# mfkiwl/msckf_stereo_c

Measured on AMD Instinct MI355X. Metric: stereo frames/sec/node on EuRoC-shape input; ATE RMSE vs CPU ref, higher is better.
Workload: dtype f64

## Files before the change

### msckf_stereo_c_amd/csrc/hip/ekf_linalg.hip

```cpp
#include <mutex>
#include <type_traits>
#include "ekf_device.h"
#include "ekf_cap.h"
#include "chol_block.h"

typedef double v4f64 __attribute__((ext_vector_type(4)));

__device__ __forceinline__ bool ekf_direct_wanted(const EkfStreamDev &S) { return ekf_mode_direct(S.qr_mode, S.rows_out[EKF_ROWS_STACKED], S.rows_out[EKF_ROWS_NA]); }
__device__ __forceinline__ bool ekf_skip_gram(const EkfStreamDev &S) { return ekf_mode_householder(S.qr_mode) || ekf_direct_wanted(S); }
__device__ __forceinline__ bool ekf_direct(const EkfStreamDev &S) { return (S.rows_out[EKF_ROWS_DIAG] & EKF_DIAG_DIRECT) != 0; }
__device__ __forceinline__ bool ekf_row_has(unsigned long long rm, int clone) { return clone < 0 ? rm != 0ULL : ((rm >> clone) & 1ULL) != 0ULL; }

template <int MODE> struct GemmTraits;
template <> struct GemmTraits<GM_GRAM> { static constexpr bool TA = true,  SYM = true,  KMIN_I = false, KMIN_J = false; };
template <> struct GemmTraits<GM_T>    { static constexpr bool TA = true,  SYM = false, KMIN_I = true,  KMIN_J = false; };
template <> struct GemmTraits<GM_S2>   { static constexpr bool TA = false, SYM = true,  KMIN_I = false, KMIN_J = true;  };
template <> struct GemmTraits<GM_PUPD> { static constexpr bool TA = true,  SYM = true,  KMIN_I = false, KMIN_J = false; };

#define GT EKF_GEMM_TILE
#ifndef GK
#define GK 32
#endif
#define GNE (GK / 8)

template <int MODE>
__global__ __launch_bounds__(256) void k_ekf_gemm(const EkfStreamDev *streams) {
    using TR = GemmTraits<MODE>;
    const EkfStreamDev &S = streams[blockIdx.y];
    if (S.n_feat <= 0) return;
    if (MODE != GM_PUPD && (S.route & EKF_ROUTE_SMALL)) return;
    const int d = S.d, ld = S.ld;
    int gram_tile_i = 0, gram_tile_j = 0;
    EkfCapResult cap = {0, 0, 0, 0ULL};
    if (MODE == GM_GRAM) {
        int tg = 1;
        while ((tg + 1) * (tg + 1) <= (int)gridDim.x) ++tg;
        gram_tile_i = (int)blockIdx.x / tg; gram_tile_j = (int)blockIdx.x - gram_tile_i * tg;
        if (gram_tile_j > gram_tile_i || gram_tile_i * GT > S.na_max) return;
        cap = ekf_cap_local(S, blockIdx.x == 0);
        if (ekf_mode_householder(S.qr_mode) || ekf_mode_direct(S.qr_mode, cap.stacked, cap.na)) return;
    }
    const int na = MODE == GM_GRAM ? cap.na : S.rows_out[EKF_ROWS_NA];
    const int *__restrict__ act = S.act;
    const double *__restrict__ A; const double *__restrict__ B; double *C;
    int M, N, K;
    double alpha = 1.0, beta = 0.0, diag_add = 0.0;
    if (MODE == GM_GRAM)      { A = S.Hs; B = S.Hs; C = S.S; M = N = na + 1; K = cap.end; }
    const int nk = MODE == GM_GRAM ? 0 : S.rows_out[EKF_ROWS_NK];
    const bool direct = MODE != GM_GRAM && MODE != GM_PUPD && ekf_direct(S);
    if (MODE == GM_T)         { A = direct ? S.Hs : S.S;  B = S.P;  C = S.T; M = nk; N = d; K = na; }
    else if (MODE == GM_S2)   { A = S.T;  B = direct ? S.Hs : S.S;  C = S.W; M = N = nk; K = na; diag_add = S.sigma2; }
    else if (MODE == GM_PUPD) { A = S.T;  B = S.T;  C = S.P; M = N = d; K = nk; alpha = -1.0; beta = 1.0; }
    const int tiles_n = (N + GT - 1) / GT, tiles_m = (M + GT - 1) / GT;
    const int tile = blockIdx.x;
    if (MODE == GM_PUPD && tile >= tiles_m * tiles_n) {
        const int c0 = (tile - tiles_m * tiles_n) * GT;
        if (c0 >= d) return;
        const double *Y = S.T;
        __shared__ double s_part[8][GT + 1];
        const int cl = threadIdx.x & 31, ks = threadIdx.x >> 5;
        const int c = c0 + cl;
        double s2 = 0;
        if (c < d)
            for (int k = ks; k < nk; k += 8) s2 += Y[(size_t)k * ld + c] * Y[(size_t)k * ld + d];
        s_part[ks][cl] = s2;
        __syncthreads();
        if (ks == 0 && c < d) {
            double t = 0;
#pragma unroll
            for (int q = 0; q < 8; ++q) t += s_part[q][cl];
            S.delta_x[c] = t;
        }
        return;
    }
    if (MODE != GM_GRAM && tile >= tiles_m * tiles_n) return;
    const int ti = MODE == GM_GRAM ? gram_tile_i : tile / tiles_n, tj = MODE == GM_GRAM ? gram_tile_j : tile - ti * tiles_n;
    if (MODE == GM_GRAM && ti >= tiles_m) return;
    if (TR::SYM && tj > ti) return;
    const int i0 = ti * GT, j0 = tj * GT;
    __shared__ double sA[GK][GT + 1];
    __shared__ double sB[GK][GT + 1];
    const int tid = threadIdx.x, lane = tid & 63, wave = tid >> 6;
    const int wi = (wave >> 1) * 16, wj = (wave & 1) * 16;
    const int lo = tid & 31, hi = tid >> 5;
    int k_begin = 0;
    if (TR::KMIN_I && !direct) k_begin = (i0 / GK) * GK;
    if (TR::KMIN_J && !direct) k_begin = (j0 / GK) * GK;
    const int k_end = K;
    int colA = i0 + lo, colB = j0 + lo;
    if (MODE == GM_GRAM) {
        colA = (i0 + lo < na) ? ekf_act_column(cap.clones, i0 + lo) : d;
        colB = (j0 + lo < na) ? ekf_act_column(cap.clones, j0 + lo) : d;
    }
    const int cloneA = MODE == GM_GRAM ? (colA < d ? (colA - EKF_IMU_DIM) / 6 : -1) : 0;
    const int cloneB = MODE == GM_GRAM ? (colB < d ? (colB - EKF_IMU_DIM) / 6 : -1) : 0;
    const unsigned long long *__restrict__ rowmask = S.rowmask;
    const int *__restrict__ rowidx = S.act + S.ld;
    double ra[GNE], rb[GNE];
    auto fetch = [&](int k0) {
#pragma unroll
        for (int e = 0; e < GNE; ++e) {
            if (MODE == GM_GRAM) {
                const int gk = k0 + hi + 8 * e;
                double v = 0.0, w = 0.0;
                if (gk < K) {
                    const unsigned long long rm = rowmask[gk];
                    const bool onA = ekf_row_has(rm, cloneA), onB = ekf_row_has(rm, cloneB);
                    if (onA && i0 + lo < M) v = A[(size_t)gk * ld + colA];
                    if (onB && j0 + lo < N) w = B[(size_t)gk * ld + colB];
                }
                ra[e] = v; rb[e] = w;
                continue;
            }
            const int ii = TR::TA ? lo : hi + 8 * (e / (GK / 32)), kk = TR::TA ? hi + 8 * e : lo + 32 * (e % (GK / 32));
            const int gi = i0 + ii, gk = k0 + kk;
            double v = 0.0;
            if (gi < M && gk < K && !(TR::KMIN_I && !direct && gk < gi)) {
                if (MODE == GM_S2) v = A[(size_t)gi * ld + act[gk]];
                else if (MODE == GM_T && direct) {
                    const int col = act[gk], ri = rowidx[gi];
                    if ((rowmask[ri] >> ((col - EKF_IMU_DIM) / 6)) & 1ULL) v = A[(size_t)ri * ld + col];
                }
                else v = A[(size_t)gk * ld + (MODE == GM_GRAM ? colA : gi)];
            }
            ra[e] = v;
            const int gj = j0 + lo, gkb = k0 + hi + 8 * e;
            double w = 0.0;
            if (gj < N && gkb < K && !(TR::KMIN_J && !direct && gkb < gj)) {
                if (MODE == GM_T) w = B[(size_t)act[gkb] * ld + gj];
                else if (MODE == GM_S2 && direct) {
                    const int col = act[gkb], rj = rowidx[gj];
                    if ((rowmask[rj] >> ((col - EKF_IMU_DIM) / 6)) & 1ULL) w = B[(size_t)rj * ld + col];
                }
                else w = B[(size_t)gkb * ld + (MODE == GM_GRAM ? colB : gj)];
            }
            rb[e] = w;
        }
    };
    v4f64 acc = {0.0, 0.0, 0.0, 0.0};
    if (k_begin < k_end) fetch(k_begin);
    for (int k0 = k_begin; k0 < k_end; k0 += GK) {
        __syncthreads();
#pragma unroll
        for (int e = 0; e < GNE; ++e) {
            if (TR::TA) sA[hi + 8 * e][lo] = ra[e]; else sA[lo + 32 * (e % (GK / 32))][hi + 8 * (e / (GK / 32))] = ra[e];
            sB[hi + 8 * e][lo] = rb[e];
        }
        __syncthreads();
        if (k0 + GK < k_end) fetch(k0 + GK);
#pragma unroll
        for (int s = 0; s < GK / 4; ++s) {
            const int kk = 4 * s + (lane >> 4);
            const double a = sA[kk][wi + (lane & 15)];
            const double b = sB[kk][wj + (lane & 15)];
            acc = __builtin_amdgcn_mfma_f64_16x16x4f64(a, b, acc, 0, 0, 0);
        }
    }
#pragma unroll
    for (int r = 0; r < 4; ++r) {
        const int i = i0 + wi + (lane >> 4) + 4 * r;
        const int j = j0 + wj + (lane & 15);
        if (i >= M || j >= N) continue;
        if (TR::SYM && j > i) continue;
        double v = alpha * acc[r];
        if (MODE == GM_PUPD) v += beta * C[(size_t)i * ld + j];
        if (i == j) v += diag_add;
        C[(size_t)i * ld + j] = v;
        if (TR::SYM && i != j) C[(size_t)j * ld + i] = v;
        if (MODE == GM_PUPD && i == j && i >= 12 && i < 15 && S.pos_var_out) S.pos_var_out[i - 12] = v;
    }
}

template <int Q> __device__ __forceinline__ double qr_lane_sum(double v) {
    auto bfly = [](double x, auto ctrl) {
        const long long b = __double_as_longlong(x);
        const int lo = __builtin_amdgcn_update_dpp(0, (int)b, decltype(ctrl)::value, 0xf, 0xf, true);
        const int hi = __builtin_amdgcn_update_dpp(0, (int)(b >> 32), decltype(ctrl)::value, 0xf, 0xf, true);
        return x + __longlong_as_double(((long long)hi << 32) | (unsigned int)lo);
    };
    v = bfly(v, std::integral_constant<int, 0xB1>());
    v = bfly(v, std::integral_constant<int, 0x4E>());
    if (Q == 8) v = bfly(v, std::integral_constant<int, 0x141>());
    return v;
}
template <int Q, int RL, class ColOf, class RAt>
__device__ __forceinline__ void tsqr_wide(const EkfStreamDev &S, int n1, int K, ColOf colOf, RAt Rat, double *sB) {
    constexpr int BR = Q * RL;
    const int tid = threadIdx.x, nth = blockDim.x, ld = S.ld;
    const int q = tid & (Q - 1), g = tid / Q, ng = nth / Q;
    for (int k0 = 0; k0 < K; k0 += BR) {
        __syncthreads();
        for (int e = tid; e < BR * n1; e += nth) {
            const int r = e / n1, c = e - r * n1, gk = k0 + r;
            double v = 0.0;
            if (gk < K) {
                int col, clone;
                colOf(c, col, clone);
                if (ekf_row_has(S.rowmask[gk], clone)) v = S.Hs[(size_t)gk * ld + col];
            }
            sB[e] = v;
        }
        __syncthreads();
        double *own = sB + (size_t)q * RL * n1;
        for (int k = 0; k < n1; ++k) {
            double bk[RL];
            double ss = 0.0;
#pragma unroll
            for (int i = 0; i < RL; ++i) { bk[i] = own[i * n1 + k]; ss += bk[i] * bk[i]; }
            ss = qr_lane_sum<Q>(ss);
            const double x0 = Rat(k, k);
            if (ss < 1e-200 || ss < 1e-40 * (x0 * x0)) continue;
            const double nrm = sqrt(x0 * x0 + ss);
            const double alpha = x0 > 0.0 ? -nrm : nrm;
            const double v0 = x0 - alpha;
            const double beta = 2.0 / (v0 * v0 + ss);
            for (int j = k + 1 + g; j < n1; j += ng) {
                double bj[RL];
                double dot = 0.0;
#pragma unroll
                for (int i = 0; i < RL; ++i) { bj[i] = own[i * n1 + j]; dot += bk[i] * bj[i]; }
                const double rkj = Rat(k, j);
                const double t = beta * (qr_lane_sum<Q>(dot) + v0 * rkj);
#pragma unroll
                for (int i = 0; i < RL; ++i) own[i * n1 + j] = bj[i] - t * bk[i];
                if (q == 0) Rat(k, j) = rkj - t * v0;
            }
            __syncthreads();
            if (tid == 0) Rat(k, k) = alpha;
        }
    }
    __syncthreads();
}
template <class ColOf, class RAt>
__device__ __forceinline__ void tsqr_quads(const EkfStreamDev &S, int n1, int K, ColOf colOf, RAt Rat, double *sB, int room) {
    if (room >= 48 * n1) tsqr_wide<4, 12>(S, n1, K, colOf, Rat, sB);
    else if (room >= 32 * n1) tsqr_wide<4, 8>(S, n1, K, colOf, Rat, sB);
    else tsqr_wide<4, 4>(S, n1, K, colOf, Rat, sB);
}

__device__ __forceinline__ int ekf_compress_entry(const EkfStreamDev &S, int *s_w ) {
    const int na = S.rows_out[EKF_ROWS_NA], me = S.rows_out[EKF_ROWS_END], d = S.d, ld = S.ld;
    if (na <= 0) { if (threadIdx.x == 0) S.rows_out[EKF_ROWS_DIAG] = 0; return 1; }
    if (ekf_direct_wanted(S)) {
        int *rowidx = S.act + ld;
        const int tid = threadIdx.x, lane = tid & 63, wave = tid >> 6, nw = (int)blockDim.x >> 6;
        int base = 0;
        for (int r0 = 0; r0 < me; r0 += (int)blockDim.x) {
            const int r = r0 + tid;
            const bool on = r < me && S.rowmask[r] != 0ULL;
            const unsigned long long b = __ballot(on);
            if (lane == 0) s_w[wave] = __popcll(b);
            __syncthreads();
            int off = base, tot = 0;
            for (int w = 0; w < nw; ++w) { const int c = s_w[w]; if (w < wave) off += c; tot += c; }
            if (on && off + __popcll(b & ((1ULL << lane) - 1ULL)) < ld) rowidx[off + __popcll(b & ((1ULL << lane) - 1ULL))] = r;
            base += tot;
            __syncthreads();
        }
        __threadfence_block();
        __syncthreads();
        for (int i = tid; i < base; i += (int)blockDim.x) S.T[(size_t)i * ld + d] = S.Hs[(size_t)rowidx[i] * ld + d];
        if (tid == 0) { S.rows_out[EKF_ROWS_DIAG] = EKF_DIAG_DIRECT; S.rows_out[EKF_ROWS_NK] = base; }
        return 1;
    }
    return ekf_skip_gram(S) ? 2 : 0;
}
template <class RAt>
__device__ __forceinline__ void ekf_hand_over_r(const EkfStreamDev &S, int na, RAt Rat, int diag) {
    const int tid = threadIdx.x, nth = blockDim.x, d = S.d, ld = S.ld;
    for (int e = tid; e < na * na; e += nth) {
        const int i = e / na, j = e - i * na;
        if (j <= i) S.S[(size_t)i * ld + j] = Rat(j, i);
    }
    for (int k = tid; k < na; k += nth) S.T[(size_t)k * ld + d] = Rat(k, na);
    if (tid == 0) S.rows_out[EKF_ROWS_DIAG] = diag | EKF_DIAG_HOUSEHOLDER;
}
template <class RAt>
__device__ __forceinline__ void ekf_compress_exit(const EkfStreamDev &S, bool gram_done, int diag, RAt Rat, double *sB, int room) {
    const int na = S.rows_out[EKF_ROWS_NA], n1 = na + 1, K = S.rows_out[EKF_ROWS_END], d = S.d;
    const int tid = threadIdx.x, nth = blockDim.x;
    if (!ekf_mode_redo_householder(S.qr_mode, gram_done, (diag & EKF_DIAG_BIAS) != 0)) { if (tid == 0) S.rows_out[EKF_ROWS_DIAG] = diag; return; }
    __syncthreads();
    for (int e = tid; e < n1 * n1; e += nth) { const int k = e / n1, j = e - k * n1; if (j >= k) Rat(k, j) = 0.0; }
    const int *act = S.act;
    tsqr_quads(S, n1, K, [=](int c, int &col, int &clone) { col = c < na ? act[c] : d; clone = c < na ? (col - EKF_IMU_DIM) / 6 : -1; }, Rat, sB, room);
    ekf_hand_over_r(S, na, Rat, diag);
}


__device__ __forceinline__ double tq_rows_sum(double v) {
    {
        const unsigned long long b = (unsigned long long)__double_as_longlong(v);
        const auto lo = __builtin_amdgcn_permlane16_swap((unsigned)b, (unsigned)b, false, false), hi = __builtin_amdgcn_permlane16_swap((unsigned)(b >> 32), (unsigned)(b >> 32), false, false);
        v = __longlong_as_double((long long)(((unsigned long long)hi[0] << 32) | lo[0])) + __longlong_as_double((long long)(((unsigned long long)hi[1] << 32) | lo[1]));
    }
    {
        const unsigned long long b = (unsigned long long)__double_as_longlong(v);
        const auto lo = __builtin_amdgcn_permlane32_swap((unsigned)b, (unsigned)b, false, false), hi = __builtin_amdgcn_permlane32_swap((unsigned)(b >> 32), (unsigned)(b >> 32), false, false);
        v = __longlong_as_double((long long)(((unsigned long long)hi[0] << 32) | lo[0])) + __longlong_as_double((long long)(((unsigned long long)hi[1] << 32) | lo[1]));
    }
    return v;
}
__device__ __forceinline__ double tq_rcp(double x) {
    double r = __builtin_amdgcn_rcp(x);
    r = __builtin_fma(__builtin_fma(-x, r, 1.0), r, r);
    r = __builtin_fma(__builtin_fma(-x, r, 1.0), r, r);
    return r;
}
template <int C, bool FIRST> __device__ __forceinline__ void tq_fmac_bcast(double &acc, double x, double a) {
    if (FIRST) asm("s_nop 4\n\tv_fmac_f64_dpp %0, %1, %2 row_newbcast:%3 row_mask:0xf bank_mask:0xf" : "+v"(acc) : "v"(x), "v"(a), "n"(C));
    else asm("v_fmac_f64_dpp %0, %1, %2 row_newbcast:%3 row_mask:0xf bank_mask:0xf" : "+v"(acc) : "v"(x), "v"(a), "n"(C));
}
template <int RL, int I = 0> struct TqDot {
    static __device__ __forceinline__ void run(double (&p)[4], const double (&vr)[RL / 16], const double (&bc)[RL]) {
        tq_fmac_bcast<I % 16, I == 0>(p[I & 3], vr[I / 16], bc[I]);
        TqDot<RL, I + 1>::run(p, vr, bc);
    }
// ... 439 lines not shown
    int pi[2], pj[2], pg[2];
    double acc[2] = {0.0, 0.0};
    for (int q = 0; q < 2; ++q) {
        int p = tid + 256 * q, grp = 0;
        if (groups > 1) { grp = q == 0 ? tid / np : groups; p = tid - grp * np; }
        pg[q] = (groups > 1) ? (grp < groups ? grp : -1) : (p < np ? 0 : -1);
        if (pg[q] < 0) p = 0;
        int i = 0;
        while ((i + 1) * (i + 2) / 2 <= p) ++i;
        pi[q] = i; pj[q] = p - i * (i + 1) / 2;
    }
    for (int k0 = 0; k0 < K; k0 += SU_CH) {
        __syncthreads();
        for (int e = tid; e < SU_CH * n1; e += 256) {
            const int r = e / n1, c = e - r * n1, gk = k0 + r;
            double v = 0.0;
            if (gk < K) {
                if (ekf_row_has(S.rowmask[gk], s_clone[c])) v = S.Hs[(size_t)gk * ld + s_col[c]];
            }
            sC[e] = v;
        }
        __syncthreads();
        for (int q = 0; q < 2; ++q) {
            if (pg[q] < 0) continue;
            double a = acc[q];
            for (int r = pg[q]; r < SU_CH; r += groups) a += sC[r * n1 + pi[q]] * sC[r * n1 + pj[q]];
            acc[q] = a;
        }
    }
    __syncthreads();
    if (groups > 1) {
        if (pg[0] >= 0) sC[pg[0] * np + (pi[0] * (pi[0] + 1) / 2 + pj[0])] = acc[0];
        __syncthreads();
        if (pg[0] == 0) {
            const int p = pi[0] * (pi[0] + 1) / 2 + pj[0];
            double t = 0.0;
            for (int g2 = 0; g2 < groups; ++g2) t += sC[g2 * np + p];
            sG[pi[0] * n1 + pj[0]] = t; sG[pj[0] * n1 + pi[0]] = t;
        }
    } else {
        for (int q = 0; q < 2; ++q)
            if (pg[q] >= 0) { sG[pi[q] * n1 + pj[q]] = acc[q]; sG[pj[q] * n1 + pi[q]] = acc[q]; }
    }
    __syncthreads();
    if (tid == 0) { double mx = 0; for (int i = 0; i < na; ++i) mx = fmax(mx, sG[i * n1 + i]); s_lam = gram_lambda(mx, d); }
    __syncthreads();
    if (tid < na) sG[tid * n1 + tid] += s_lam;
    __syncthreads();
    su_chol(sG, n1, na, n1);
    if (tid == 0) {
        int t = 0;
        double pm = 0;
        for (int i = 0; i < na; ++i) {
            t += gram_tiny_pivot(sG[i * n1 + i], s_lam) ? 1 : 0;
            pm = fmax(pm, S.P[(size_t)s_col[i] * ld + s_col[i]]);
        }
        s_tiny = t;
        s_bias = gram_biased(s_lam, pm, S.sigma2) ? 1 : 0;
    }
    }
    {
        __syncthreads();
        const int diag = ekf_diag_encode(s_tiny, s_bias != 0);
        const bool need_qr = ekf_mode_redo_householder(S.qr_mode, cap.stacked > na, (diag & EKF_DIAG_BIAS) != 0);
        if (need_qr) {
            for (int e = tid; e < n1 * n1; e += 256) sG[e] = 0.0;
            __syncthreads();
            static_assert(SU_CH == 128 && SU_MAX_NA + 1 <= 32, "tsqr_wave<32, 2>: 128-row blocks, two 16-column slabs");
            {
                const int wv = __builtin_amdgcn_readfirstlane(tid >> 6);
                double *sRw = sC;
                double *sVq = (double *)(((uintptr_t)(sC + 3 * n1 * n1) + 15) & ~(uintptr_t)15);
                int *sFq = (int *)(sVq + 4 * 130);
                for (int e = tid; e < 3 * n1 * n1; e += 256) sRw[e] = 0.0;
                __syncthreads();
                const unsigned long long *rowmask = S.rowmask;
                const double *Hs = S.Hs;
                auto loadH = [&](int blk, int row, int col) -> double {
                    const int gk = blk * 128 + row;
                    if (gk >= K || col >= n1) return 0.0;
                    return ekf_row_has(rowmask[gk], s_clone[col]) ? Hs[(size_t)gk * ld + s_col[col]] : 0.0;
                };
                double *Rmine = wv == 0 ? sG : sRw + (wv - 1) * n1 * n1;
                tsqr_wave<32, 2>(n1, (K + 127) / 128, wv, 4, loadH, Rmine, n1, sVq + wv * 130, sFq + wv);
                __syncthreads();
                if (wv == 0) {
                    auto loadR = [&](int, int row, int col) -> double {
                        if (row >= 3 * n1 || col >= n1) return 0.0;
                        const int w2 = row / n1, rr = row - w2 * n1;
                        return col >= rr ? sRw[(w2 * n1 + rr) * n1 + col] : 0.0;
                    };
                    tsqr_wave<32, 2>(n1, 1, 0, 1, loadR, sG, n1, sVq, sFq);
                }
                __syncthreads();
            }
            for (int e = tid; e < n1 * n1; e += 256) { const int i = e / n1, j = e - i * n1; if (j < i) sG[e] = sG[j * n1 + i]; }
            __syncthreads();
        }
        if (tid == 0) S.rows_out[EKF_ROWS_DIAG] = diag | (need_qr ? EKF_DIAG_HOUSEHOLDER : 0);
    }
    const double *P = S.P;
    for (int c = tid; c < d; c += 256) {
        double pc[SU_MAX_NA];
#pragma unroll
        for (int k = 0; k < SU_MAX_NA; ++k) pc[k] = k < na ? P[(size_t)s_col[k] * ld + c] : 0.0;
#pragma unroll
        for (int i = 0; i < SU_MAX_NA; ++i) {
            if (i < na) {
                double t = 0.0;
#pragma unroll
                for (int k = i; k < SU_MAX_NA; ++k) if (k < na) t += sG[k * n1 + i] * pc[k];
                sT[i * (d + 1) + c] = t;
            }
        }
    }
    if (tid < na) sT[tid * (d + 1) + d] = sG[na * n1 + tid];
    __syncthreads();
    for (int e = tid; e < na * na; e += 256) {
        const int i = e / na, j = e - i * na;
        if (j > i) continue;
        double t = 0.0;
        for (int k = j; k < na; ++k) t += sT[i * (d + 1) + s_col[k]] * sG[k * n1 + j];
        if (i == j) t += S.sigma2;
        sS[i * na + j] = t; sS[j * na + i] = t;
    }
    __syncthreads();
    su_chol(sS, na, na, na);
    for (int c = tid; c <= d; c += 256) {
        double y[SU_MAX_NA];
#pragma unroll
        for (int i = 0; i < SU_MAX_NA; ++i) {
            y[i] = 0.0;
            if (i >= na) continue;
            double t = sT[i * (d + 1) + c];
#pragma unroll
            for (int k = 0; k < i; ++k) t -= sS[i * na + k] * y[k];
            const double l = sS[i * na + i];
            y[i] = l != 0.0 ? t / l : 0.0;
            sT[i * (d + 1) + c] = y[i];
        }
    }
    __syncthreads();
    for (int e = tid; e < na * (d + 1); e += 256) {
        const int k = e / (d + 1), c = e - k * (d + 1);
        S.T[(size_t)k * ld + c] = sT[e];
    }
}

extern "C" {
void ekf_launch_gemm(const EkfStreamDev *d, int n, int mode, int max_mn, hipStream_t st) {
    const int t = (max_mn + GT - 1) / GT;
    const dim3 grid(t * t + (mode == GM_PUPD ? t : 0), n);
    switch (mode) {
        case GM_GRAM: hipLaunchKernelGGL(k_ekf_gemm<GM_GRAM>, grid, dim3(256), 0, st, d); break;
        case GM_T:    hipLaunchKernelGGL(k_ekf_gemm<GM_T>, grid, dim3(256), 0, st, d); break;
        case GM_S2:   hipLaunchKernelGGL(k_ekf_gemm<GM_S2>, grid, dim3(256), 0, st, d); break;
        default:      hipLaunchKernelGGL(k_ekf_gemm<GM_PUPD>, grid, dim3(256), 0, st, d); break;
    }
}
void ekf_launch_tsqr(const EkfStreamDev *d, int n, int min_d, int max_d, int do_cap, hipStream_t st) {
    const int lo = tsqr_class(min_d), hi = tsqr_class(max_d), cls = lo == hi ? -1 : 0;
    if (lo == 0) hipLaunchKernelGGL((k_ekf_tsqr<32, 2, 2>), dim3(1, n), dim3(TQ_THREADS), 0, st, d, do_cap, cls);
    if (hi == 1) hipLaunchKernelGGL((k_ekf_tsqr<16, 4, 2>), dim3(1, n), dim3(TQ_THREADS), 0, st, d, do_cap, lo == hi ? -1 : 1);
}
void ekf_launch_chol(const EkfStreamDev *d, int n, int which, int min_d, int max_d, hipStream_t st) {
    const int lo = chol_class(min_d), hi = chol_class(max_d);
    if (lo == 0) {
        static std::once_flag attr_once;
        std::call_once(attr_once, []() { (void)hipFuncSetAttribute(reinterpret_cast<const void *>(k_ekf_chol_lds), hipFuncAttributeMaxDynamicSharedMemorySize,
                                      (int)(((size_t)CHOL_LDS_MAX_ROWS * (CHOL_LDS_MAX_ROWS + 1) / 2 + (size_t)CHOL_PAN_RS * LNB) * sizeof(double))); });
        const size_t lds = (size_t)chol_lds_doubles(hi == 0 ? max_d : EKF_IMU_DIM + CHOL_LDS_MAX_ROWS - 1) * sizeof(double);
        hipLaunchKernelGGL(k_ekf_chol_lds, dim3(1, n), dim3(CHOL_THREADS), lds, st, d, which, lo == hi ? -1 : 0);
    }
    if (hi == 1) {
        const int nt = max_d - EKF_IMU_DIM + 1;
        const int pan_rs = (nt + 15) / 16 * 16;
        hipLaunchKernelGGL(k_ekf_chol, dim3(1, n), dim3(CHOL_THREADS), (size_t)LNB * pan_rs * sizeof(double), st, d, which, pan_rs, lo == hi ? -1 : 1);
    }
}
void ekf_launch_small_update(const EkfStreamDev *d, int n, int max_d, hipStream_t st) {
    const size_t lds = ((size_t)SU_MAX_NA * (max_d + 1) + (SU_MAX_NA + 1) * (SU_MAX_NA + 1) + SU_MAX_NA * SU_MAX_NA + SU_CH * (SU_MAX_NA + 1)) * sizeof(double);
    static std::once_flag attr_once;
    std::call_once(attr_once, []() {
        hipFuncAttributes fa;
        size_t stat = 4096;
        if (hipFuncGetAttributes(&fa, reinterpret_cast<const void *>(k_ekf_small_update)) == hipSuccess) stat = fa.sharedSizeBytes;
        if (hipFuncSetAttribute(reinterpret_cast<const void *>(k_ekf_small_update), hipFuncAttributeMaxDynamicSharedMemorySize, (int)(160 * 1024 - stat)) != hipSuccess) (void)hipGetLastError();
    });
    hipLaunchKernelGGL(k_ekf_small_update, dim3(1, n), dim3(256), lds, st, d);
}
void ekf_launch_trsm(const EkfStreamDev *d, int n, int max_d, hipStream_t st) {
    const int strips = (max_d + 1 + TS_COLS - 1) / TS_COLS;
    const int max_n = max_d > EKF_IMU_DIM ? max_d - EKF_IMU_DIM : 1;
    const size_t lds = (size_t)(TS_RB * (max_n + 1) + (size_t)max_n * TS_COLS) * sizeof(double);
    static std::once_flag attr_once;
    std::call_once(attr_once, []() { (void)hipFuncSetAttribute(reinterpret_cast<const void *>(k_ekf_trsm), hipFuncAttributeMaxDynamicSharedMemorySize, 160 * 1024); });
    hipLaunchKernelGGL(k_ekf_trsm, dim3(strips, n), dim3(256), lds, st, d);
}
}
```

### msckf_stereo_c_amd/csrc/hip/fe_kernels.hip

```cpp
#include <stdlib.h>
#include <mutex>
#include "fe_device.h"

__device__ __forceinline__ int reflect101(int i, int n) {
    if (n == 1) return 0;
    while (i < 0 || i >= n) { i = (i < 0) ? -i : 2 * (n - 1) - i; }
    return i;
}

#define P3_HALO 2
#define P3_OWN 12
#define P3_SEG_ROWS 8
struct Pyr3Job { const uint8_t *src; uint8_t *d1, *d2, *d3; int w0, h0; };

namespace {
typedef uint32_t __attribute__((aligned(1))) pd_u32u;
typedef uint16_t __attribute__((aligned(1))) pd_u16u;
typedef unsigned long long __attribute__((aligned(1))) pd_u64u;
typedef const __attribute__((address_space(1))) pd_u64u *pd_gld64;
typedef __attribute__((address_space(1))) pd_u32u *pd_gst32;
typedef __attribute__((address_space(1))) pd_u16u *pd_gst16;
typedef __attribute__((address_space(1))) uint8_t *pd_gst8;

template <int CTRL> __device__ __forceinline__ uint32_t pd_dpp0(uint32_t v) { return (uint32_t)__builtin_amdgcn_update_dpp(0, (int)v, CTRL, 0xf, 0xf, true); }
// ... 982 lines not shown
    const int nch = (x1 - x0 + 15) / 16 + 1, n_items = (yb - ya) * nch;
    for (int idx = tid; idx < n_items; idx += 256) {
        const int rr = idx / nch, ch = idx - rr * nch, y = ya + rr;
        const size_t row = (size_t)y * w, pb = row + x0, pe = row + x1;
        const size_t P = (pb & ~(size_t)15) + 16 * (size_t)ch;
        if (P >= pe) continue;
        const int lo = pb > P ? (int)(pb - P) : 0, hi = pe - P < 16 ? (int)(pe - P) : 16;
        const bool whole = lo == 0 && hi == 16;
        uint32_t in[4] = {0u, 0u, 0u, 0u}, out[4] = {0u, 0u, 0u, 0u};
        if (whole) { const eq_u4 v = *reinterpret_cast<const eq_u4 *>(j.src + P); in[0] = v.v[0]; in[1] = v.v[1]; in[2] = v.v[2]; in[3] = v.v[3]; }
        else {
#pragma unroll
            for (int k = 0; k < 16; ++k) if (k >= lo && k < hi) in[k >> 2] |= (uint32_t)j.src[P + k] << (8 * (k & 3));
        }
        EqAxis ay = {0, 0, 0.f, 0.f};
        if (clahe) ay = eq_axis(y, inv_th, j.tiles_y);
        const int xb = (int)(P - row);
#pragma unroll
        for (int k = 0; k < 16; ++k) {
            const uint32_t v = (in[k >> 2] >> (8 * (k & 3))) & 255u, L = s_lut[v];
            uint32_t o = L;
            if (clahe) {
                const EqAxis ax = eq_axis(xb + k, inv_tw, j.tiles_x);
                o = (uint32_t)eq_interp((int)(L & 255u), (int)((L >> 8) & 255u), (int)((L >> 16) & 255u), (int)(L >> 24), ax.a, ax.a1, ay.a, ay.a1);
            }
            out[k >> 2] |= o << (8 * (k & 3));
        }
        if (whole) *reinterpret_cast<uint4 *>(j.dst + P) = make_uint4(out[0], out[1], out[2], out[3]);
        else {
#pragma unroll
            for (int k = 0; k < 16; ++k) if (k >= lo && k < hi) j.dst[P + k] = (uint8_t)(out[k >> 2] >> (8 * (k & 3)));
        }
    }
}

extern "C" void fe_launch_equalize(const EqJob *jobs_dev, int n_jobs, int max_units, int any_global, int max_regions, int splits, hipStream_t st) {
    if (n_jobs <= 0) return;
    hipLaunchKernelGGL(k_eq_hist, dim3(max_units, n_jobs), dim3(256), 0, st, jobs_dev);
    if (any_global) hipLaunchKernelGGL(k_eq_lut, dim3(n_jobs), dim3(256), 0, st, jobs_dev);
    hipLaunchKernelGGL(k_eq_apply, dim3(max_regions * splits, n_jobs), dim3(256), 0, st, jobs_dev, splits);
}

#include "fe_pixfmt.h"
namespace {
#if defined(__HIP_DEVICE_COMPILE__)
#define PX_GLOBAL __attribute__((address_space(1)))
#else
#define PX_GLOBAL
#endif
typedef const PX_GLOBAL uint8_t *px_gptr;
__device__ __forceinline__ px_gptr px_global(const uint8_t *p) { return (px_gptr)(uintptr_t)p; }
__device__ __forceinline__ uint32_t px_byte(const uint32_t *v, int i) { return (v[i >> 2] >> (8 * (i & 3))) & 255u; }
template <int NV>
__device__ __forceinline__ void px_load(uint32_t *v, px_gptr p) {
#pragma unroll
    for (int q = 0; q < NV; ++q) {
        const eq_u4 t = *reinterpret_cast<const PX_GLOBAL eq_u4 *>(p + 16 * q);
        v[4 * q] = t.v[0]; v[4 * q + 1] = t.v[1]; v[4 * q + 2] = t.v[2]; v[4 * q + 3] = t.v[3];
    }
}
template <int FMT>
__device__ __forceinline__ void px_chunk16(const PxJob &j, int x0, int y, uint32_t out[4]) {
    out[0] = out[1] = out[2] = out[3] = 0u;
    constexpr int BPP = FMT == PX_GRAY16 ? 2 : (FMT == PX_RGB8 || FMT == PX_BGR8) ? 3 : 4;
    uint32_t v[4 * BPP];
    px_load<BPP>(v, px_global(j.src) + (size_t)y * (size_t)j.pitch + (size_t)x0 * BPP);
#pragma unroll
    for (int k = 0; k < 16; ++k) {
        int g;
        if (FMT == PX_GRAY16) g = px_gray16((int)((v[k >> 1] >> (16 * (k & 1))) & 0xFFFFu), j.shift);
        else {
            const int c0 = (int)px_byte(v, BPP * k), c1 = (int)px_byte(v, BPP * k + 1), c2 = (int)px_byte(v, BPP * k + 2);
            g = (FMT == PX_RGB8 || FMT == PX_RGBA8) ? px_luma(c0, c1, c2) : px_luma(c2, c1, c0);
        }
        out[k >> 2] |= (uint32_t)g << (8 * (k & 3));
    }
}
__device__ __forceinline__ void px_chunk16_bayer(const PxJob &j, int x0, int y, uint32_t out[4]) {
    out[0] = out[1] = out[2] = out[3] = 0u;
    const px_gptr src = px_global(j.src);
    const px_gptr rows[3] = {src + (size_t)px_reflect(y - 1, j.h) * (size_t)j.pitch + x0, src + (size_t)y * (size_t)j.pitch + x0,
                             src + (size_t)px_reflect(y + 1, j.h) * (size_t)j.pitch + x0};
    uint32_t v[3][4], lft[3], rgt[3];
#pragma unroll
    for (int r = 0; r < 3; ++r) { px_load<1>(v[r], rows[r]); lft[r] = rows[r][-1]; rgt[r] = rows[r][16]; }
    const int site0 = px_bayer_site(j.format, x0, y), site1 = px_bayer_site(j.format, x0 + 1, y);
#pragma unroll
    for (int k = 0; k < 16; ++k) {
        int a[3], b[3], c[3];
#pragma unroll
        for (int r = 0; r < 3; ++r) {
            a[r] = (int)(k == 0 ? lft[r] : px_byte(v[r], k - 1));
            b[r] = (int)px_byte(v[r], k);
            c[r] = (int)(k == 15 ? rgt[r] : px_byte(v[r], k + 1));
        }
        const int g = px_bayer_luma((k & 1) ? site1 : site0, b[1], a[1], c[1], b[0], b[2], a[0], c[0], a[2], c[2]);
        out[k >> 2] |= (uint32_t)g << (8 * (k & 3));
    }
}
template <int FMT>
__device__ __forceinline__ void px_rows(const PxJob &j) {
    const int w = j.w, h = j.h;
    const int nch = (w + 15) / 16 + 1;
    const long long n_items = (long long)h * nch;
    for (long long idx = (long long)blockIdx.x * 256 + threadIdx.x; idx < n_items; idx += (long long)gridDim.x * 256) {
        const int y = (int)(idx / nch), ch = (int)(idx - (long long)y * nch);
        const uintptr_t pb = (uintptr_t)j.dst + (size_t)y * w, pe = pb + (size_t)w;
        const uintptr_t P = (pb & ~(uintptr_t)15) + 16 * (uintptr_t)ch;
        if (P >= pe) continue;
        const int lo = pb > P ? (int)(pb - P) : 0, hi = pe - P < 16 ? (int)(pe - P) : 16;
        const int x0 = (int)((long long)P - (long long)pb);
        bool whole = lo == 0 && hi == 16;
        if (FMT == PX_BAYER_RGGB8) whole = whole && x0 >= 1 && x0 + 16 <= w - 1;
        if (whole) {
            uint32_t out[4];
            if (FMT == PX_BAYER_RGGB8) px_chunk16_bayer(j, x0, y, out); else px_chunk16<FMT>(j, x0, y, out);
            *reinterpret_cast<PX_GLOBAL uint4 *>(P) = make_uint4(out[0], out[1], out[2], out[3]);
        } else {
            for (int k = lo; k < hi; ++k) *reinterpret_cast<PX_GLOBAL uint8_t *>(P + k) = (uint8_t)px_pixel(j.src, (size_t)j.pitch, w, h, j.format, j.shift, x0 + k, y);
        }
    }
}
}

__global__ __launch_bounds__(256) void k_px_convert(const PxJob *jobs) {
    const PxJob j = jobs[blockIdx.y];
    switch (j.format) {
        case PX_GRAY16: px_rows<PX_GRAY16>(j); break;
        case PX_RGB8: px_rows<PX_RGB8>(j); break;
        case PX_BGR8: px_rows<PX_BGR8>(j); break;
        case PX_RGBA8: px_rows<PX_RGBA8>(j); break;
        case PX_BGRA8: px_rows<PX_BGRA8>(j); break;
        case PX_BAYER_RGGB8: case PX_BAYER_GRBG8: case PX_BAYER_GBRG8: case PX_BAYER_BGGR8: px_rows<PX_BAYER_RGGB8>(j); break;
        default: break;
    }
}

extern "C" void fe_launch_px_convert(const PxJob *jobs_dev, int n_jobs, int max_w, int max_h, hipStream_t st) {
    if (n_jobs <= 0 || max_w <= 0 || max_h <= 0) return;
    const long long items = (long long)max_h * ((max_w + 15) / 16 + 1);
    const long long wgs = (items + 255) / 256;
    hipLaunchKernelGGL(k_px_convert, dim3((unsigned)(wgs > 65535 ? 65535 : wgs), n_jobs), dim3(256), 0, st, jobs_dev);
}

__global__ void k_mark(volatile unsigned int *flag, unsigned int seq) {
    *flag = seq;
    __threadfence_system();
}
extern "C" void fe_launch_mark(volatile unsigned int *flag, unsigned int seq, hipStream_t st) {
    hipLaunchKernelGGL(k_mark, dim3(1), dim3(1), 0, st, flag, seq);
}

struct MskfCopySegs { void *dst[MSKF_COPY_SEGS]; const void *src[MSKF_COPY_SEGS]; unsigned long long bytes[MSKF_COPY_SEGS]; int blocks_per_seg; };
__global__ __launch_bounds__(256) void k_mskf_copy(MskfCopySegs segs) {
    const int seg = (int)blockIdx.x / segs.blocks_per_seg, b = (int)blockIdx.x - seg * segs.blocks_per_seg;
    const unsigned long long bytes = segs.bytes[seg], n16 = bytes >> 4;
    const uint4 *__restrict__ src = (const uint4 *)segs.src[seg];
    uint4 *__restrict__ dst = (uint4 *)segs.dst[seg];
    const unsigned long long stride = (unsigned long long)segs.blocks_per_seg * 256ULL;
    unsigned long long i = (unsigned long long)b * 256ULL + threadIdx.x;
    for (; i + 3ULL * stride < n16; i += 4ULL * stride) {
        const uint4 a0 = src[i], a1 = src[i + stride], a2 = src[i + 2ULL * stride], a3 = src[i + 3ULL * stride];
        dst[i] = a0; dst[i + stride] = a1; dst[i + 2ULL * stride] = a2; dst[i + 3ULL * stride] = a3;
    }
    for (; i < n16; i += stride) dst[i] = src[i];
    if (b == 0 && threadIdx.x < (unsigned)(bytes & 15ULL)) ((uint8_t *)dst)[(n16 << 4) + threadIdx.x] = ((const uint8_t *)src)[(n16 << 4) + threadIdx.x];
}
extern "C" void fe_launch_copy(void *const *dst, const void *const *src, const size_t *bytes, int n_segs, hipStream_t st) {
    MskfCopySegs segs;
    size_t mx = 0;
    for (int i = 0; i < MSKF_COPY_SEGS; ++i) {
        segs.dst[i] = i < n_segs ? dst[i] : nullptr; segs.src[i] = i < n_segs ? src[i] : nullptr; segs.bytes[i] = i < n_segs ? bytes[i] : 0ULL;
        if (i < n_segs && bytes[i] > mx) mx = bytes[i];
    }
    if (n_segs <= 0 || mx == 0) return;
    size_t bps = (mx + 16383) / 16384;
    segs.blocks_per_seg = (int)(bps < 1 ? 1 : bps > 96 ? 96 : bps);
    hipLaunchKernelGGL(k_mskf_copy, dim3(segs.blocks_per_seg * n_segs), dim3(256), 0, st, segs);
}

extern "C" void fe_launch_track(const FeStreamDev *streams_dev, int n_streams, int max_pts, hipStream_t st) {
    if (max_pts <= 0) return;
    const int gps = (max_pts + 3) / 4;
    hipLaunchKernelGGL(k_track4, dim3(8 * ((n_streams + 7) / 8) * gps), dim3(64), 0, st, streams_dev, n_streams, gps);
}
```

Measured before the change: 106,200.

## Rewrite EKF GEMM as single-wave register-fed MFMA tiles and retune copy kernel

The EKF GEMM kernel goes from four waves staging tiles through shared memory to a single 64-thread wave. That wave computes the whole 32x32 tile as four 16x16 MFMA accumulators fed straight from registers, with a register double-buffered prefetch and no __syncthreads. The delta_x reduction tail now uses a shuffle instead of shared memory, and the segmented copy kernel moves to 64-thread groups with an 8-way unrolled loop and more blocks. The aim is to cut LDS traffic and barrier cost in the small f64 GEMMs. In exchange each lane holds more registers, and per-wave loads are no longer reused across waves through LDS.

```diff
diff --git a/msckf_stereo_c_amd/csrc/hip/ekf_linalg.hip b/msckf_stereo_c_amd/csrc/hip/ekf_linalg.hip
--- a/msckf_stereo_c_amd/csrc/hip/ekf_linalg.hip
+++ b/msckf_stereo_c_amd/csrc/hip/ekf_linalg.hip
@@ -18,13 +18,15 @@
 template <> struct GemmTraits<GM_PUPD> { static constexpr bool TA = true,  SYM = true,  KMIN_I = false, KMIN_J = false; };
 
 #define GT EKF_GEMM_TILE
+#define GKB 32
 #ifndef GK
-#define GK 32
+#define GK 16
 #endif
-#define GNE (GK / 8)
+#define GNC (GK / 4)
+static_assert(GKB % GK == 0 && GK % 4 == 0, "a GKB range is a whole number of stages, a stage a whole number of MFMA chunks");
 
 template <int MODE>
-__global__ __launch_bounds__(256) void k_ekf_gemm(const EkfStreamDev *streams) {
+__global__ __launch_bounds__(64) __attribute__((amdgpu_waves_per_eu(4))) void k_ekf_gemm(const EkfStreamDev *streams) {
     using TR = GemmTraits<MODE>;
     const EkfStreamDev &S = streams[blockIdx.y];
     if (S.n_feat <= 0) return;
@@ -37,7 +39,7 @@
         while ((tg + 1) * (tg + 1) <= (int)gridDim.x) ++tg;
         gram_tile_i = (int)blockIdx.x / tg; gram_tile_j = (int)blockIdx.x - gram_tile_i * tg;
         if (gram_tile_j > gram_tile_i || gram_tile_i * GT > S.na_max) return;
-        cap = ekf_cap_local(S, blockIdx.x == 0);
+        cap = ekf_cap_local<64>(S, blockIdx.x == 0);
         if (ekf_mode_householder(S.qr_mode) || ekf_mode_direct(S.qr_mode, cap.stacked, cap.na)) return;
     }
     const int na = MODE == GM_GRAM ? cap.na : S.rows_out[EKF_ROWS_NA];
@@ -57,20 +59,21 @@
         const int c0 = (tile - tiles_m * tiles_n) * GT;
         if (c0 >= d) return;
         const double *Y = S.T;
-        __shared__ double s_part[8][GT + 1];
-        const int cl = threadIdx.x & 31, ks = threadIdx.x >> 5;
+        const int cl = threadIdx.x & 31, kh = 4 * (int)(threadIdx.x >> 5);
         const int c = c0 + cl;
-        double s2 = 0;
+        double part[4] = {0.0, 0.0, 0.0, 0.0};
         if (c < d)
-            for (int k = ks; k < nk; k += 8) s2 += Y[(size_t)k * ld + c] * Y[(size_t)k * ld + d];
-        s_part[ks][cl] = s2;
-        __syncthreads();
-        if (ks == 0 && c < d) {
-            double t = 0;
-#pragma unroll
-            for (int q = 0; q < 8; ++q) t += s_part[q][cl];
-            S.delta_x[c] = t;
-        }
+            for (int k = kh; k < nk; k += 8) {
+#pragma unroll
+                for (int q = 0; q < 4; ++q)
+                    if (k + q < nk) part[q] += Y[(size_t)(k + q) * ld + c] * Y[(size_t)(k + q) * ld + d];
+            }
+        double t = 0;
+#pragma unroll
+        for (int q = 0; q < 4; ++q) t += part[q];
+#pragma unroll
+        for (int q = 0; q < 4; ++q) t += __shfl_down(part[q], 32);
+        if (kh == 0 && c < d) S.delta_x[c] = t;
         return;
     }
     if (MODE != GM_GRAM && tile >= tiles_m * tiles_n) return;
@@ -78,91 +81,93 @@
     if (MODE == GM_GRAM && ti >= tiles_m) return;
     if (TR::SYM && tj > ti) return;
     const int i0 = ti * GT, j0 = tj * GT;
-    __shared__ double sA[GK][GT + 1];
-    __shared__ double sB[GK][GT + 1];
-    const int tid = threadIdx.x, lane = tid & 63, wave = tid >> 6;
-    const int wi = (wave >> 1) * 16, wj = (wave & 1) * 16;
-    const int lo = tid & 31, hi = tid >> 5;
+    const int lane = threadIdx.x, li = lane & 15, lk = lane >> 4;
     int k_begin = 0;
-    if (TR::KMIN_I && !direct) k_begin = (i0 / GK) * GK;
-    if (TR::KMIN_J && !direct) k_begin = (j0 / GK) * GK;
-    const int k_end = K;
-    int colA = i0 + lo, colB = j0 + lo;
-    if (MODE == GM_GRAM) {
-        colA = (i0 + lo < na) ? ekf_act_column(cap.clones, i0 + lo) : d;
-        colB = (j0 + lo < na) ? ekf_act_column(cap.clones, j0 + lo) : d;
-    }
-    const int cloneA = MODE == GM_GRAM ? (colA < d ? (colA - EKF_IMU_DIM) / 6 : -1) : 0;
-    const int cloneB = MODE == GM_GRAM ? (colB < d ? (colB - EKF_IMU_DIM) / 6 : -1) : 0;
+    if (TR::KMIN_I && !direct) k_begin = (i0 / GKB) * GKB;
+    if (TR::KMIN_J && !direct) k_begin = (j0 / GKB) * GKB;
+    const int k_end = K > k_begin ? k_begin + (K - k_begin + GKB - 1) / GKB * GKB : k_begin;
     const unsigned long long *__restrict__ rowmask = S.rowmask;
     const int *__restrict__ rowidx = S.act + S.ld;
-    double ra[GNE], rb[GNE];
-    auto fetch = [&](int k0) {
-#pragma unroll
-        for (int e = 0; e < GNE; ++e) {
+    int gi[2], gj[2], colA[2], colB[2], cloneA[2], cloneB[2], rowA[2], rowB[2];
+    unsigned long long rmA[2], rmB[2];
+#pragma unroll
+    for (int h = 0; h < 2; ++h) {
+        gi[h] = i0 + 16 * h + li; gj[h] = j0 + 16 * h + li;
+        colA[h] = gi[h]; colB[h] = gj[h]; cloneA[h] = cloneB[h] = 0; rowA[h] = rowB[h] = 0; rmA[h] = rmB[h] = 0ULL;
+        if (MODE == GM_GRAM) {
+            colA[h] = gi[h] < na ? ekf_act_column(cap.clones, gi[h]) : d;
+            colB[h] = gj[h] < na ? ekf_act_column(cap.clones, gj[h]) : d;
+            cloneA[h] = colA[h] < d ? (colA[h] - EKF_IMU_DIM) / 6 : -1;
+            cloneB[h] = colB[h] < d ? (colB[h] - EKF_IMU_DIM) / 6 : -1;
+        }
+        if (MODE == GM_T && direct && gi[h] < M) { rowA[h] = rowidx[gi[h]]; rmA[h] = rowmask[rowA[h]]; }
+        if (MODE == GM_S2 && direct && gj[h] < N) { rowB[h] = rowidx[gj[h]]; rmB[h] = rowmask[rowB[h]]; }
+    }
+    auto fetch = [&](int k0, double (&ra)[GNC][2], double (&rb)[GNC][2]) {
+#pragma unroll
+        for (int c = 0; c < GNC; ++c) {
+            const int gk = k0 + 4 * c + lk;
+            const bool kin = gk < K;
             if (MODE == GM_GRAM) {
-                const int gk = k0 + hi + 8 * e;
-                double v = 0.0, w = 0.0;
-                if (gk < K) {
-                    const unsigned long long rm = rowmask[gk];
-                    const bool onA = ekf_row_has(rm, cloneA), onB = ekf_row_has(rm, cloneB);
-                    if (onA && i0 + lo < M) v = A[(size_t)gk * ld + colA];
-                    if (onB && j0 + lo < N) w = B[(size_t)gk * ld + colB];
+                const unsigned long long rm = kin ? rowmask[gk] : 0ULL;
+#pragma unroll
+                for (int h = 0; h < 2; ++h) {
+                    double v = 0.0, w = 0.0;
+                    if (kin && gi[h] < M && ekf_row_has(rm, cloneA[h])) v = A[(size_t)gk * ld + colA[h]];
+                    if (kin && gj[h] < N && ekf_row_has(rm, cloneB[h])) w = B[(size_t)gk * ld + colB[h]];
+                    ra[c][h] = v; rb[c][h] = w;
                 }
-                ra[e] = v; rb[e] = w;
                 continue;
             }
-            const int ii = TR::TA ? lo : hi + 8 * (e / (GK / 32)), kk = TR::TA ? hi + 8 * e : lo + 32 * (e % (GK / 32));
-            const int gi = i0 + ii, gk = k0 + kk;
-            double v = 0.0;
-            if (gi < M && gk < K && !(TR::KMIN_I && !direct && gk < gi)) {
-                if (MODE == GM_S2) v = A[(size_t)gi * ld + act[gk]];
-                else if (MODE == GM_T && direct) {
-                    const int col = act[gk], ri = rowidx[gi];
-                    if ((rowmask[ri] >> ((col - EKF_IMU_DIM) / 6)) & 1ULL) v = A[(size_t)ri * ld + col];
+            const int ak = (kin && (MODE == GM_T || MODE == GM_S2)) ? act[gk] : EKF_IMU_DIM;
+#pragma unroll
+            for (int h = 0; h < 2; ++h) {
+                double v = 0.0;
+                if (gi[h] < M && kin && !(TR::KMIN_I && !direct && gk < gi[h])) {
+                    if (MODE == GM_S2) v = A[(size_t)gi[h] * ld + ak];
+                    else if (MODE == GM_T && direct) {
+                        if ((rmA[h] >> ((ak - EKF_IMU_DIM) / 6)) & 1ULL) v = A[(size_t)rowA[h] * ld + ak];
+                    }
+                    else v = A[(size_t)gk * ld + gi[h]];
                 }
-                else v = A[(size_t)gk * ld + (MODE == GM_GRAM ? colA : gi)];
-            }
-            ra[e] = v;
-            const int gj = j0 + lo, gkb = k0 + hi + 8 * e;
-            double w = 0.0;
-            if (gj < N && gkb < K && !(TR::KMIN_J && !direct && gkb < gj)) {
-                if (MODE == GM_T) w = B[(size_t)act[gkb] * ld + gj];
-                else if (MODE == GM_S2 && direct) {
-                    const int col = act[gkb], rj = rowidx[gj];
-                    if ((rowmask[rj] >> ((col - EKF_IMU_DIM) / 6)) & 1ULL) w = B[(size_t)rj * ld + col];
+                ra[c][h] = v;
+                double w = 0.0;
+                if (gj[h] < N && kin && !(TR::KMIN_J && !direct && gk < gj[h])) {
+                    if (MODE == GM_T) w = B[(size_t)ak * ld + gj[h]];
+                    else if (MODE == GM_S2 && direct) {
+                        if ((rmB[h] >> ((ak - EKF_IMU_DIM) / 6)) & 1ULL) w = B[(size_t)rowB[h] * ld + ak];
+                    }
+                    else w = B[(size_t)gk * ld + gj[h]];
                 }
-                else w = B[(size_t)gkb * ld + (MODE == GM_GRAM ? colB : gj)];
-            }
-            rb[e] = w;
+                rb[c][h] = w;
+            }
         }
     };
-    v4f64 acc = {0.0, 0.0, 0.0, 0.0};
-    if (k_begin < k_end) fetch(k_begin);
+    v4f64 acc[2][2];
+#pragma unroll
+    for (int h = 0; h < 4; ++h) acc[h >> 1][h & 1] = (v4f64){0.0, 0.0, 0.0, 0.0};
+    double na_[GNC][2], nb_[GNC][2];
+    if (k_begin < k_end) fetch(k_begin, na_, nb_);
     for (int k0 = k_begin; k0 < k_end; k0 += GK) {
-        __syncthreads();
-#pragma unroll
-        for (int e = 0; e < GNE; ++e) {
-            if (TR::TA) sA[hi + 8 * e][lo] = ra[e]; else sA[lo + 32 * (e % (GK / 32))][hi + 8 * (e / (GK / 32))] = ra[e];
-            sB[hi + 8 * e][lo] = rb[e];
-        }
-        __syncthreads();
-        if (k0 + GK < k_end) fetch(k0 + GK);
-#pragma unroll
-        for (int s = 0; s < GK / 4; ++s) {
-            const int kk = 4 * s + (lane >> 4);
-            const double a = sA[kk][wi + (lane & 15)];
-            const double b = sB[kk][wj + (lane & 15)];
-            acc = __builtin_amdgcn_mfma_f64_16x16x4f64(a, b, acc, 0, 0, 0);
-        }
-    }
-#pragma unroll
-    for (int r = 0; r < 4; ++r) {
-        const int i = i0 + wi + (lane >> 4) + 4 * r;
-        const int j = j0 + wj + (lane & 15);
+        double ra[GNC][2], rb[GNC][2];
+#pragma unroll
+        for (int c = 0; c < GNC; ++c) { ra[c][0] = na_[c][0]; ra[c][1] = na_[c][1]; rb[c][0] = nb_[c][0]; rb[c][1] = nb_[c][1]; }
+        if (k0 + GK < k_end) fetch(k0 + GK, na_, nb_);
+#pragma unroll
+        for (int c = 0; c < GNC; ++c)
+#pragma unroll
+            for (int h = 0; h < 4; ++h)
+                acc[h >> 1][h & 1] = __builtin_amdgcn_mfma_f64_16x16x4f64(ra[c][h >> 1], rb[c][h & 1], acc[h >> 1][h & 1], 0, 0, 0);
+    }
+#pragma unroll
+    for (int q = 0; q < 16; ++q) {
+        const int h = q >> 2, r = q & 3, wi = (h >> 1) * 16, wj = (h & 1) * 16;
+        const int i = i0 + wi + lk + 4 * r;
+        const int j = j0 + wj + li;
+        const v4f64 &accq = acc[h >> 1][h & 1];
         if (i >= M || j >= N) continue;
         if (TR::SYM && j > i) continue;
-        double v = alpha * acc[r];
+        double v = alpha * accq[r];
         if (MODE == GM_PUPD) v += beta * C[(size_t)i * ld + j];
         if (i == j) v += diag_add;
         C[(size_t)i * ld + j] = v;
@@ -908,10 +913,10 @@
     const int t = (max_mn + GT - 1) / GT;
     const dim3 grid(t * t + (mode == GM_PUPD ? t : 0), n);
     switch (mode) {
-        case GM_GRAM: hipLaunchKernelGGL(k_ekf_gemm<GM_GRAM>, grid, dim3(256), 0, st, d); break;
-        case GM_T:    hipLaunchKernelGGL(k_ekf_gemm<GM_T>, grid, dim3(256), 0, st, d); break;
-        case GM_S2:   hipLaunchKernelGGL(k_ekf_gemm<GM_S2>, grid, dim3(256), 0, st, d); break;
-        default:      hipLaunchKernelGGL(k_ekf_gemm<GM_PUPD>, grid, dim3(256), 0, st, d); break;
+        case GM_GRAM: hipLaunchKernelGGL(k_ekf_gemm<GM_GRAM>, grid, dim3(64), 0, st, d); break;
+        case GM_T:    hipLaunchKernelGGL(k_ekf_gemm<GM_T>, grid, dim3(64), 0, st, d); break;
+        case GM_S2:   hipLaunchKernelGGL(k_ekf_gemm<GM_S2>, grid, dim3(64), 0, st, d); break;
+        default:      hipLaunchKernelGGL(k_ekf_gemm<GM_PUPD>, grid, dim3(64), 0, st, d); break;
     }
 }
 void ekf_launch_tsqr(const EkfStreamDev *d, int n, int min_d, int max_d, int do_cap, hipStream_t st) {
diff --git a/msckf_stereo_c_amd/csrc/hip/fe_kernels.hip b/msckf_stereo_c_amd/csrc/hip/fe_kernels.hip
--- a/msckf_stereo_c_amd/csrc/hip/fe_kernels.hip
+++ b/msckf_stereo_c_amd/csrc/hip/fe_kernels.hip
@@ -1158,13 +1158,22 @@
 }
 
 struct MskfCopySegs { void *dst[MSKF_COPY_SEGS]; const void *src[MSKF_COPY_SEGS]; unsigned long long bytes[MSKF_COPY_SEGS]; int blocks_per_seg; };
-__global__ __launch_bounds__(256) void k_mskf_copy(MskfCopySegs segs) {
+#define COPY_WG 64
+#define COPY_SWEEP (COPY_WG * 16 * 4)
+#define COPY_MAX_BLOCKS 384
+__global__ __launch_bounds__(COPY_WG) void k_mskf_copy(MskfCopySegs segs) {
     const int seg = (int)blockIdx.x / segs.blocks_per_seg, b = (int)blockIdx.x - seg * segs.blocks_per_seg;
     const unsigned long long bytes = segs.bytes[seg], n16 = bytes >> 4;
     const uint4 *__restrict__ src = (const uint4 *)segs.src[seg];
     uint4 *__restrict__ dst = (uint4 *)segs.dst[seg];
-    const unsigned long long stride = (unsigned long long)segs.blocks_per_seg * 256ULL;
-    unsigned long long i = (unsigned long long)b * 256ULL + threadIdx.x;
+    const unsigned long long stride = (unsigned long long)segs.blocks_per_seg * COPY_WG;
+    unsigned long long i = (unsigned long long)b * COPY_WG + threadIdx.x;
+    for (; i + 7ULL * stride < n16; i += 8ULL * stride) {
+        const uint4 a0 = src[i], a1 = src[i + stride], a2 = src[i + 2ULL * stride], a3 = src[i + 3ULL * stride];
+        const uint4 a4 = src[i + 4ULL * stride], a5 = src[i + 5ULL * stride], a6 = src[i + 6ULL * stride], a7 = src[i + 7ULL * stride];
+        dst[i] = a0; dst[i + stride] = a1; dst[i + 2ULL * stride] = a2; dst[i + 3ULL * stride] = a3;
+        dst[i + 4ULL * stride] = a4; dst[i + 5ULL * stride] = a5; dst[i + 6ULL * stride] = a6; dst[i + 7ULL * stride] = a7;
+    }
     for (; i + 3ULL * stride < n16; i += 4ULL * stride) {
         const uint4 a0 = src[i], a1 = src[i + stride], a2 = src[i + 2ULL * stride], a3 = src[i + 3ULL * stride];
         dst[i] = a0; dst[i + stride] = a1; dst[i + 2ULL * stride] = a2; dst[i + 3ULL * stride] = a3;
@@ -1180,9 +1189,9 @@
         if (i < n_segs && bytes[i] > mx) mx = bytes[i];
     }
     if (n_segs <= 0 || mx == 0) return;
-    size_t bps = (mx + 16383) / 16384;
-    segs.blocks_per_seg = (int)(bps < 1 ? 1 : bps > 96 ? 96 : bps);
-    hipLaunchKernelGGL(k_mskf_copy, dim3(segs.blocks_per_seg * n_segs), dim3(256), 0, st, segs);
+    size_t bps = (mx + COPY_SWEEP - 1) / COPY_SWEEP;
+    segs.blocks_per_seg = (int)(bps < 1 ? 1 : bps > COPY_MAX_BLOCKS ? COPY_MAX_BLOCKS : bps);
+    hipLaunchKernelGGL(k_mskf_copy, dim3(segs.blocks_per_seg * n_segs), dim3(COPY_WG), 0, st, segs);
 }
 
 extern "C" void fe_launch_track(const FeStreamDev *streams_dev, int n_streams, int max_pts, hipStream_t st) {
```

After: 104,200. 0.982x the previous value.
